# sdrobert/pydrobert-speech

Measured on AMD Instinct MI355X. Metric: frames/s (whole node) + HBM-roofline %, 40-mel fbank 16kHz 25/10ms, higher is better.
Workload: dtype f32

## Files before the change

include/pds_amd.h:

```cpp
#ifndef PDS_AMD_H
#define PDS_AMD_H

#include <stdint.h>

#ifdef __cplusplus
extern "C" {
#endif

#define PDS_OK 0
#define PDS_ERR_INVALID -1
#define PDS_ERR_HIP -2
#define PDS_ERR_NOMEM -3

int32_t pds_version(void);
int32_t pds_build_experiments(void);
const char *pds_last_error(void);
int32_t pds_device_count(void);

typedef struct pds_stft_desc {
  int32_t frame_length;
  int32_t frame_shift;
  int32_t dft_size;
  int32_t pad_left;
  int32_t num_filts;
  int32_t nnz;
  int32_t use_power;
  int32_t use_log;
  int32_t include_energy;
  int32_t reserved;
  double log_floor;
// ... 237 lines not shown
```

pydrobert-speech_amd/_native.py:

```python
import ctypes
import os
from ctypes import POINTER, Structure, c_char_p, c_double, c_int32, c_int64, c_void_p

_HERE = os.path.dirname(os.path.abspath(__file__))
LIB_PATH = os.environ.get("PDS_AMD_LIB") or os.path.join(_HERE, "csrc", "libpds_amd.so")

PDS_OK = 0


class NativeError(RuntimeError):
    """A call into libpds_amd.so failed"""


class StftDesc(Structure):
    _fields_ = [
        ("frame_length", c_int32),
        ("frame_shift", c_int32),
        ("dft_size", c_int32),
        ("pad_left", c_int32),
        ("num_filts", c_int32),
        ("nnz", c_int32),
        ("use_power", c_int32),
        ("use_log", c_int32),
        ("include_energy", c_int32),
# ... 41 lines not shown
    c_void_p, c_int64, c_int64, c_int64,
    c_void_p, c_void_p, c_int32,
    c_int32, c_int32,
    c_void_p, c_int64, c_int64, c_int64, c_int64,
    c_void_p,
]

_CMVN_ROWS_ARGS = [
    c_void_p, c_int64, c_void_p, c_void_p, c_int32, c_int32, c_int32,
    c_void_p, c_void_p, c_int64, c_void_p, c_void_p,
]

SIGNATURES = {
    "pds_version": (c_int32, []),
    "pds_build_experiments": (c_int32, []),
    "pds_last_error": (c_char_p, []),
    "pds_device_count": (c_int32, []),
    "pds_stft_plan_create": (
        c_int32,
        [POINTER(StftDesc), c_void_p, c_void_p, c_void_p, c_void_p, POINTER(c_void_p)],
    ),
    "pds_stft_plan_destroy": (None, [c_void_p]),
    "pds_stft_num_coeffs": (c_int32, [c_void_p]),
    "pds_stft_num_frames": (c_int64, [c_void_p, c_int64]),
    "pds_stft_plan_kernel_kind": (c_int32, [c_void_p]),
    "pds_stft_plan_filter_walk": (c_int32, [c_void_p]),
    "pds_stft_batch_f32": (c_int32, _BATCH_ARGS),
    "pds_stft_batch_f64": (c_int32, _BATCH_ARGS),
    "pds_stft_batch_f32_generic": (c_int32, _BATCH_ARGS),
    "pds_stft_plan_has_f64in": (c_int32, [c_void_p]),
# ... 148 lines not shown
```

pydrobert-speech_amd/csrc/stft_fast.hip:

```cpp
#include "stft_wave_launch.h"

namespace pds {

#if PDS_STAMPS
unsigned long long *g_stamp_buf = nullptr;
extern "C" __attribute__((visibility("default"))) void pds_debug_set_stamp_buffer(unsigned long long *d_buf) {
  g_stamp_buf = d_buf;
}
#endif

extern "C" __attribute__((visibility("default"))) int32_t pds_build_experiments(void) { return PDS_EXPERIMENTS ? 1 : 0; }

bool fast_has_f64in(const pds_stft_plan *plan) { return plan->fast.kind && fast_f64in_kind(plan->fast.kind); }

bool fast_has_fused_cmvn(const pds_stft_plan *plan) {
  const FastTables &ft = plan->fast;
  return ft.kind && ft.n2 == 16 && ((ft.n1 == 64 && ft.walk != 0) || (ft.n1 == 32 && (ft.walk == 1 || ft.walk == 3)));
}

bool fast_has_fused_deltas(const pds_stft_plan *plan) {
  const FastTables &ft = plan->fast;
  return ft.kind && fast_deltas_kind(ft.kind) && ft.rsn_rounds >= 1 && ft.rsn_rounds <= 2 &&
         (!plan->d.include_energy || ft.rs_eslot >= 0);
}

__global__ __launch_bounds__(1024) void chunk_prefix_kernel(const int64_t *nframes, int B, int groups, int64_t *prefix) {
// ... 382 lines not shown
```

pydrobert-speech_amd/csrc/stft_wave_kernel.h:

```cpp
#pragma once
#include <algorithm>
#include <atomic>
#include <cmath>
#include <cstdio>
#include <cstdlib>
#include <cstring>
#include <type_traits>
#include <vector>

#include "fft_inlane.h"
#include "mfma_front.h"
#include "rseg_tables.h"
#include "mseg_tables.h"
#include "pds_internal.h"

#include "stft_switches.h"

namespace pds {

__device__ __forceinline__ void keep_alive(float v) { asm volatile("" ::"v"(v)); }

struct FastParams {
  const void *sig;
  const int64_t *offsets, *lengths, *nframes, *row_off;
  void *out;
  int64_t out_stride;
  const float *win_lane;
  const float2 *tw_lane;
// ... 64 lines not shown
  typedef const T __attribute__((address_space(4))) *const_ptr;
  return *(const_ptr)(uintptr_t)ptr;
}

template <int CTRL>
__device__ __forceinline__ float dpp_add(float x) {
  return x + __int_as_float(__builtin_amdgcn_update_dpp(0, __float_as_int(x), CTRL, 0xf, 0xf, false));
}

__device__ __forceinline__ void wave_sync() {
  __builtin_amdgcn_fence(__ATOMIC_RELEASE, "wavefront");
  __builtin_amdgcn_wave_barrier();
  __builtin_amdgcn_fence(__ATOMIC_ACQUIRE, "wavefront");
}

#ifndef PDS_TWOPASS
#define PDS_TWOPASS 1
#endif
#ifndef PDS_LEAN_2048
#define PDS_LEAN_2048 1
#endif
constexpr bool lean_geometry(int n1, int n2) { return PDS_LEAN_2048 && n1 == 64 && n2 == 32; }
constexpr int wave_area_floats(int n1, int n2) {
  const int cols = (n1 - 1) / 2 + 1, groups = 64 / n2, one_pass = groups * cols * (n2 + 2) * 2;
  return (PDS_TWOPASS && n1 == 64 && n2 == 16) ? 2688 : lean_geometry(n1, n2) ? groups * cols * (n2 + 4) : one_pass;
}
constexpr int win_table_stride(int rows) { return ((rows + 3) & ~3) % 8 == 4 ? ((rows + 3) & ~3) : ((rows + 3) & ~3) + 4; }

template <int N1, int N2, int NROWS>
struct WaveGeom {
// ... 21 lines not shown
  static_assert(inl::is_pow2(N1) ? (FULL || N2 == 2 * COLS) : 600 % N1 == 0,
                "in-lane DFT sizes: 2^k, or a divisor of 600");
  static_assert(NROWS <= N1 && NROWS > 0, "rows");
};

constexpr int USLOTS = 4;

typedef float f32x4 __attribute__((ext_vector_type(4)));

template <int N1, int N2, int NROWS, int MAXWAVES, int MINW, bool ELL_LDS, bool PRE, int SEG = 0, int MF = 0,
          bool RSG = false, typename TIN = float, typename TOUT = float, int DLT = 0, bool STR = false, bool PF = false>
__global__ __launch_bounds__(MAXWAVES * 64, MINW) void stft_wave_kernel(const FastParams p) {
  static_assert(!PF || (DLT == 0 && !STR && MF == 0 && !PRE && std::is_same<TIN, float>::value && (N1 == 32 || N1 == 64) && N2 == 16),
                "prefetch: 16-lane power-of-two geometries, float32 samples, round-robin scheduling");
  constexpr bool STRETCH = DLT > 0 || STR;
  static_assert(!(STR && DLT > 0), "stretch scheduling is part of the fused-deltas launches already");
  static_assert(DLT == 0 || (DLT == 2 && N2 == 16 && RSG && std::is_same<TOUT, float>::value && MF == 0),
                "fused deltas: row-segment walk, float32 features");
  static_assert(MF == 0 || std::is_same<TIN, float>::value, "matrix-pipe front end: float32 samples");
  static_assert(std::is_same<TIN, float>::value || std::is_same<TIN, double>::value || std::is_same<TIN, int16_t>::value, "samples: float32, float64 or int16");
  using G = WaveGeom<N1, N2, NROWS>;
  constexpr int N = G::N, COLS = G::COLS, NREG = G::NREG, RS = G::RS, NB = G::NB, PSTR = G::PSTR;
  constexpr int MSLOTS = 2 * MF + 1;
  static_assert(MF == 0 || (N2 == 16 && N1 == 32 && MF == mfma_front_steps(NROWS)), "matrix-pipe front end: 32 x 16");
  static_assert(MF == 0 || 4 * MSLOTS * 64 <= G::EXCH_F2 * 2, "edge-frame gather reuses the exchange area");
  constexpr int NBP = (NB + 3) / 4 * 4;
  static_assert(!RSG || (G::GROUPS == 4 && ELL_LDS && !SEG && (NBP + 1) * 4 <= G::EXCH_F2 * 2),
                "row-segment walk: four frames per wave, tables in LDS");
  extern __shared__ __attribute__((aligned(16))) float smem[];
  const int lane = threadIdx.x & 63;
// ... 18 lines not shown
        t2 = fma(d, d, t2);
      }
    wstat[col] += t1;
    wstat[p.stat_cs + col] += t2;
  };
  float2 *exch = reinterpret_cast<float2 *>(wbase) + g * G::XROWS * RS;
  [[maybe_unused]] float *xf = wbase + g * (G::XROWS * G::RSF);
  float *Pg = wbase + g * PSTR;
  const int nthreads = p.waves * 64;
  float2 *sw_lds = reinterpret_cast<float2 *>(smem + p.waves * p.area_f);
  int *meta_lds = reinterpret_cast<int *>(sw_lds + N2);
  float *ellw_lds = reinterpret_cast<float *>(meta_lds + p.ell_meta_pad);
  constexpr bool TWCHAIN = (PF && PDS_PF_TW == 1) || (PAIR && (N1 == 32 || N1 == 64)) || (PDS_DLT_CHAIN && DLT > 0 && N1 == 32 && N2 == 16) || G::LEAN ||
                           (N1 == 64 && N2 == 16 && (SEG == 2 || PDS_LEAN_1024));
  constexpr bool WINLDS = PF && PDS_PF_WIN == 1;
  constexpr bool WINUSE = G::LEAN || (N1 == 64 && N2 == 16 && (SEG == 2 || PDS_LEAN_1024));
  constexpr int WSTR = win_table_stride(NROWS);
  [[maybe_unused]] float *win_lds = ellw_lds + (ELL_LDS ? p.ell_wfloats : 0);
  if constexpr (WINLDS || WINUSE) {
    const float *wsrc = TWCHAIN ? p.win_half : p.win_lane;
    for (int i = threadIdx.x; i < N2 * WSTR; i += p.waves * 64) {
      const int rr = i / WSTR, k = i - rr * WSTR;
      win_lds[i] = k < NROWS ? wsrc[rr * N1 + k] : 0.0f;
    }
  }
  if (threadIdx.x < N2) sw_lds[threadIdx.x] = p.tw_special[threadIdx.x];
  constexpr bool DYN = PDS_DYN && !STRETCH && !PF;
  [[maybe_unused]] int *ticket_lds = reinterpret_cast<int *>(smem + p.lds_ticket_off);
  if constexpr (DYN) {
    if (threadIdx.x == 0) *ticket_lds = p.waves;
  }
// ... 152 lines not shown
  };
  int nfr = 0, n = 0;
  int64_t sig_off = 0, out_row = 0;
  if (!STRETCH && b < p.num_utts) {
    nfr = (int)load_const(p.nframes + b);
    n = (int)load_const(p.lengths + b);
    sig_off = load_const(p.offsets + b);
    out_row = load_const(p.row_off + b);
  }
  constexpr int DR = 2;
  [[maybe_unused]] int left = 0, e_lo = 0, e_hi = 0, c_last = -1;
  [[maybe_unused]] bool piece_open = false, ran = false;
  [[maybe_unused]] float Wp[DR][4], Wc[DR][4], e_keep = 0.0f;
  if constexpr (STRETCH) {
    const int gw = wg * p.waves + wave, GW = (int)gridDim.x * p.waves;
    const int total = (int)load_const(p.chunk_prefix + p.num_utts);
    const int per = total / GW, rem = total - per * GW;
    const int pos = gw * per + (gw < rem ? gw : rem);
    left = per + (gw < rem ? 1 : 0);
    int lo = 0, hi = p.num_utts;
    while (left > 0 && hi - lo > 1) {
      const int mid = (lo + hi) >> 1;
      if ((int)load_const(p.chunk_prefix + mid) <= pos) lo = mid; else hi = mid;
    }
    b = lo;
    e_lo = left > 0 ? pos - (int)load_const(p.chunk_prefix + lo) : 0;
    chunk = 0;
#pragma unroll
    for (int rd = 0; rd < DR; ++rd)
#pragma unroll
      for (int q = 0; q < 4; ++q) Wp[rd][q] = Wc[rd][q] = 0.0f;
  }
  [[maybe_unused]] auto emit_rows = [&](const int ce, const float (&nx)[DR][4]) {
    if (p.dl_debug & 2) return;
    const int C = p.dl_inner;
    const int W = (p.dl_order + 1) * C, WS = (W + 3) & ~3;
    float *stage = wbase;
    wave_sync();
#pragma unroll
    for (int rd = 0; rd < DR; ++rd) {
      if (rd >= p.seg_rounds) break;
// ... 46 lines not shown
                const float4 val = *reinterpret_cast<const float4 *>(stage + q * WS + 4 * l);
                F4 o = {val.x, val.y, val.z, val.w};
                *reinterpret_cast<F4 *>(orow + (int64_t)q * p.out_stride + 4 * l) = o;
              }
          }
        }
      }
      if (tail) {
        const int q = tail == 1 ? lane : tail == 2 ? lane >> 1 : (lane * 11) >> 5;
        const int jj = lane - q * tail;
        if (q < fh && q < 4) orow[(int64_t)q * p.out_stride + 4 * full + jj] = stage[q * WS + 4 * full + jj];
      }
    }
    wave_sync();
  };
  [[maybe_unused]] unsigned long long st_acc[8] = {0, 0, 0, 0, 0, 0, 0, 0};
  [[maybe_unused]] unsigned long long st_prev = PDS_STAMPS ? __builtin_readcyclecounter() : 0;
  [[maybe_unused]] const unsigned long long st_loop = st_prev;
  while (STRETCH || b < p.num_utts) {
    if constexpr (STRETCH) {
      if (!piece_open) {
        if (left <= 0) break;
        nfr = (int)load_const(p.nframes + b);
        const int chunks_b = (nfr + G::GROUPS - 1) / G::GROUPS;
        if (e_lo >= chunks_b) {
          ++b;
          e_lo = 0;
          continue;
        }
        n = (int)load_const(p.lengths + b);
        sig_off = load_const(p.offsets + b);
        out_row = load_const(p.row_off + b);
        e_hi = e_lo + left < chunks_b ? e_lo + left : chunks_b;
        c_last = DLT > 0 ? (e_hi < chunks_b ? e_hi : chunks_b - 1) : e_hi - 1;
        chunk = DLT > 0 ? (e_lo > 0 ? e_lo - 1 : 0) : e_lo;
        piece_open = true;
        ran = false;
      }
      if constexpr (STR) {
        if (ran) ++chunk;
        ran = true;
      }
      if (chunk > c_last) {
        if (DLT > 0 && c_last < e_hi) {
          float nx[DR][4];
#pragma unroll
          for (int rd = 0; rd < DR; ++rd)
#pragma unroll
            for (int q = 0; q < 4; ++q) nx[rd][q] = Wc[rd][3];
          emit_rows(c_last, nx);
        }
        if constexpr (STATS) {
          if (stats_on) {
            wave_sync();
            double *dst = p.stat_part + ((int64_t)(wg * p.waves + wave) + b) * (2 * p.stat_c);
            for (int c = lane; c < p.stat_c; c += 64) {
              dst[c] = wstat[c];
              dst[p.stat_c + c] = wstat[p.stat_cs + c];
              wstat[c] = 0.0;
              wstat[p.stat_cs + c] = 0.0;
            }
            wave_sync();
          }
        }
        left -= e_hi - e_lo;
        ++b;
        e_lo = 0;
        piece_open = false;
        continue;
      }
    }
    int nchunk = chunk + p.step_chunks, nb = b + p.step_utts;
    if (nchunk >= p.chunks_per_utt) {
      nchunk -= p.chunks_per_utt;
      ++nb;
    }
    const int pb = nb < p.num_utts ? nb : b;
    const int tb = chunk * G::GROUPS;
    if constexpr (DYN) {
      if (p.dyn) fetch_ticket();
// ... 29 lines not shown
      const float *base = pf_ready ? static_cast<const float *>(p.sig) + (sig_off_nx + s02) : p.win_lane;
      const float *xp2 = base + (pf_ready ? pf_lane : r);
#pragma unroll
      for (int n1 = 0; n1 < NROWS; ++n1) {
        pfv[n1] = xp2[n1 * N2];
#if PDS_PF_ILV > 0
        __builtin_amdgcn_sched_group_barrier(0x020, 1, 0);
        __builtin_amdgcn_sched_group_barrier(0x002, PDS_PF_ILV, 0);
#endif
      }
    };
    const TIN *x = static_cast<const TIN *>(p.sig) + sig_off;
    const int start0 = tb * S - p.pad_left;
    bool valid = true;
    float energy = 0.0f;
    const float2 sw = sw_lds[r];
    [[maybe_unused]] float even_sum, odd_sum, Ar[COLS], Ai[COLS];
    if constexpr (MF > 0) {
      int fstart[4];
#pragma unroll
      for (int fg = 0; fg < 4; ++fg) fstart[fg] = start0 + fg * S;
      int wmode = 0;
      if (!(tb + 4 <= nfr && start0 >= (PRE ? 1 : 0) && start0 + 3 * S + NROWS * 16 <= n)) {
        valid = tb + g < nfr;
#pragma unroll
        for (int fg = 0; fg < 4; ++fg) {
          const int st = (tb + fg < nfr ? tb + fg : nfr - 1) * S - p.pad_left;
          fstart[fg] = st;
          int mode = (st < (PRE ? 1 : 0) || st + NROWS * 16 > n) ? 1 : 0;
          if (st < -n || st + L > 2 * n) mode = 2;
          wmode = mode > wmode ? mode : wmode;
// ... 116 lines not shown
        for (int v = 0; v < 4; ++v) {
          float2 val;
          val.x = accR[fg][v] * mtwr[v] - accI[fg][v] * mtwi[v];
          val.y = accR[fg][v] * mtwi[v] + accI[fg][v] * mtwr[v];
          if (v < 3 || g != 3) {
            mine[fg * COLS * RS + v * RS] = val;
          } else {
            row0[fg * COLS * RS * 2] = accR[fg][3];
            row0[fg * COLS * RS * 2 + 16] = accI[fg][3];
          }
        }
      }
    } else {
      int start = start0 + __mul24(g, S);
      int wmode = 0;
      if (!(PF && pf_ready) && !(tb + G::GROUPS <= nfr && start0 >= (PRE ? 1 : 0) &&
            start0 + (G::GROUPS - 1) * S + LOADSPAN <= n)) {
        valid = tb + g < nfr;
        start = (valid ? tb + g : nfr - 1) * S - p.pad_left;
        int mode = 0;
        if (start < (PRE ? 1 : 0) || start + LOADSPAN > n) mode = 1;
        if (start < -n || start + L > 2 * n) mode = 2;
        wmode = __builtin_amdgcn_readfirstlane(__any(mode == 2) ? 2 : (__any(mode == 1) ? 1 : 0));
      }

      float a[N1];
      if (PF && pf_ready) {
#pragma unroll
        for (int n1 = 0; n1 < NROWS; ++n1) a[n1] = pfv[n1];
      } else if (wmode == 0) {
        const TIN *xp = x + (start + r);
        if constexpr (PAIR) {
          typedef double D2 __attribute__((ext_vector_type(2), aligned(8)));
          const TIN *xq = x + (start + 2 * r);
          constexpr int NP = (NROWS + 1) / 2;
          D2 w2[NP];
          [[maybe_unused]] double before = 0.0;
#pragma unroll
          for (int j = 0; j < NP; ++j) w2[j] = *reinterpret_cast<const D2 *>(xq + 32 * j);
          if constexpr (PRE) {
            if (r == 0) before = xq[-1];
          }
// ... 123 lines not shown
                i = (int)reflect_index((int64_t)i, (int64_t)n);
              }
              if constexpr (!F64S) {
                v = (float)x[i];
                if (PRE && i > 0) v = preemph_sample(v, (float)x[i - 1], p.preemph);
              } else {
                TIN w = x[i];
                if (PRE && i > 0) w = preemph_sample(w, x[i - 1], (TIN)p.preemph_d);
                v = (float)w;
              }
            }
            tmp[(n1 - base) * 64 + lane] = v;
          }
          wave_sync();
#pragma unroll
          for (int n1 = base; n1 < top; ++n1) a[n1] = tmp[(n1 - base) * 64 + lane];
          wave_sync();
        });
      }
      if (p.include_energy) {
        int lim = L - rho;
        asm volatile("" : "+v"(lim));
#pragma unroll
        for (int n1 = 0; n1 < NROWS; ++n1) {
          const float v = (n1 < N1 / 2 || n1 * N2 < lim) ? a[n1] : 0.0f;
          energy = fmaf(v, v, energy);
        }
      }
      PDS_STAMP(0, 0);
      PDS_STAMP(1, 1);
      PDS_PHASE(4);
      if constexpr (WINLDS) {
#pragma unroll
        for (int n1 = 0; n1 < NROWS; ++n1) a[n1] = window_mul<N1>(n1, a[n1], wl[n1]);
      } else if constexpr (WINUSE) {
        const float4 *w4 = reinterpret_cast<const float4 *>(win_lds + rho * WSTR);
#pragma unroll
        for (int j = 0; j < (NROWS + 3) / 4; ++j) {
          const float4 w = w4[j];
          const float wv[4] = {w.x, w.y, w.z, w.w};
#pragma unroll
          for (int u = 0; u < 4; ++u)
            if (4 * j + u < NROWS) a[4 * j + u] = window_mul<N1>(4 * j + u, a[4 * j + u], wv[u]);
        }
      } else {
#pragma unroll
        for (int n1 = 0; n1 < NROWS; ++n1) a[n1] = window_mul<N1>(n1, a[n1], win[n1]);
      }
      if constexpr (PF) fetch_next_record();
#pragma unroll
      for (int n1 = NROWS; n1 < N1; ++n1) a[n1] = 0.0f;

      if constexpr (PDS_ABLATE & 2) {
        even_sum = a[0];
        odd_sum = a[1];
#pragma unroll
        for (int k = 0; k < COLS; ++k) {
          Ar[k] = a[2 * k];
// ... 264 lines not shown
        if constexpr (G::FULL && PDS_MIRROR_REBASE) {
          float *const Pa = Pw + kk * PB, *const Pm = Pw + (N1 - kk) * PB;
#pragma unroll
          for (int k2 = 0; k2 < N2 / 2; ++k2) Pa[N1 * k2 * PB] = pw[q][k2];
#pragma unroll
          for (int k2 = N2 / 2; k2 < N2; ++k2) Pm[N1 * (N2 - 1 - k2) * PB] = pw[q][k2];
        } else
#pragma unroll
        for (int k2 = 0; k2 < N2; ++k2) {
          const int bin = (k2 < N2 / 2) ? kk + N1 * k2 : N - kk - N1 * k2;
          Pw[(live ? bin : PDUMP) * PB] = pw[q][k2];
        }
      }
    }
    if constexpr (G::DIST) {
      const bool has = r <= N2 / 2 && (N1 % 2 == 0 || r % 2 == 0);
      Pw[(has ? r * N1 / 2 : PDUMP) * PB] = sp0;
      Pw[(has ? (N2 - r) * N1 / 2 : PDUMP) * PB] = sp1;
    }
    if constexpr (RSG) {
      constexpr int PADF = (NBP - NB) * 4;
      wbase[NB * 4 + (lane < PADF ? lane : PADF - 1)] = 0.0f;
    } else {
#pragma unroll
      for (int j0 = 0; j0 < PSTR - NB; j0 += N2) {
        const int j = j0 + r;
        Pg[NB + (j < PSTR - NB ? j : PSTR - NB - 1)] = 0.0f;
      }
    }
    TOUT *obase = static_cast<TOUT *>(p.out) + (out_row + tb) * p.out_stride;
    const unsigned lane_off = (unsigned)(g * (int)p.out_stride + col0);
    if (p.include_energy) {
      if constexpr (MF == 0) {
        energy = dpp_add<0xB1>(energy);
        energy = dpp_add<0x4E>(energy);
        energy = dpp_add<0x141>(energy);
        if constexpr (N2 >= 16) energy = dpp_add<0x140>(energy);
        if constexpr (N2 >= 32) energy += __shfl_xor(energy, 16, 64);
        if constexpr (N2 == 64) energy += __shfl_xor(energy, 32, 64);
      }
      float e = energy * p.inv_L;
      if (!use_power) e = __builtin_amdgcn_sqrtf(e);
      if (p.use_log) e = floor_log(e, p.log_floor);
      if (DLT == 0 && valid && r == 0) {
        unsigned off = (lane_off - col0) * (unsigned)sizeof(TOUT);
        asm("" : "+v"(off));
        *reinterpret_cast<TOUT *>(reinterpret_cast<char *>(obase) + off) = (TOUT)e;
      }
      if constexpr (DLT > 0) e_keep = e;
      if constexpr (STATS) {
        if (stats_on) {
          const float e4[4] = {__int_as_float(__builtin_amdgcn_readlane(__float_as_int(e), 0)),
                               __int_as_float(__builtin_amdgcn_readlane(__float_as_int(e), 16)),
                               __int_as_float(__builtin_amdgcn_readlane(__float_as_int(e), 32)),
                               __int_as_float(__builtin_amdgcn_readlane(__float_as_int(e), 48))};
          if (lane == 0) stat_add4(0, e4, nfr - tb);
        }
      }
    }
    PDS_STAMP(4, 0);
// ... 71 lines not shown
      if (steps & 1u) step();
      float acc = (acc0 + acc1) + (acc2 + acc3);
      if (p.use_log) acc = floor_log(acc, p.log_floor);
      if constexpr (PDS_ABLATE & 64) {
        keep_alive(acc);
      } else {
        const unsigned byte_off = (lane_off + (unsigned)(meta >> 16) - 1u) * (unsigned)sizeof(TOUT);
        if (valid && meta >= 0x10000)
          *reinterpret_cast<TOUT *>(reinterpret_cast<char *>(obase) + byte_off) = (TOUT)acc;
      }
    };
    if constexpr (RSG) {
      const float4 *P4 = reinterpret_cast<const float4 *>(wbase);
      const int t4n = p.seg_len >> 2;
      char *const orow0 = reinterpret_cast<char *>(obase);
      const int64_t row_bytes = p.out_stride * (int64_t)sizeof(TOUT);
      auto round_body = [&](const int rd, float (&logged)[4]) {
        const int4 rec = reinterpret_cast<const int4 *>(meta_lds)[rd * 64 + lane];
        const float4 *prow = reinterpret_cast<const float4 *>(reinterpret_cast<const char *>(P4) + rec.x);
        const float4 *wrow = reinterpret_cast<const float4 *>(ellw_lds) + __mul24(rd, t4n) * 64 + lane;
        float a0 = 0.0f, a1 = 0.0f, a2 = 0.0f, a3 = 0.0f;
        auto quad = [&](int t4) {
          const float4 w = wrow[t4 * 64];
          const float4 x0 = prow[4 * t4], x1 = prow[4 * t4 + 1], x2 = prow[4 * t4 + 2], x3 = prow[4 * t4 + 3];
          a0 = fmaf(w.x, x0.x, a0);
          a1 = fmaf(w.x, x0.y, a1);
          a2 = fmaf(w.x, x0.z, a2);
          a3 = fmaf(w.x, x0.w, a3);
          a0 = fmaf(w.y, x1.x, a0);
          a1 = fmaf(w.y, x1.y, a1);
          a2 = fmaf(w.y, x1.z, a2);
// ... 41 lines not shown
                     : "+v"(a0), "+v"(a1), "+v"(a2), "+v"(a3) : "v"(m1), "v"(m2));
#else
        a0 = fmaf(shl(a0, inl::Int<0x101>{}), m1, a0);
        a1 = fmaf(shl(a1, inl::Int<0x101>{}), m1, a1);
        a2 = fmaf(shl(a2, inl::Int<0x101>{}), m1, a2);
        a3 = fmaf(shl(a3, inl::Int<0x101>{}), m1, a3);
        a0 = fmaf(shl(a0, inl::Int<0x102>{}), m2, a0);
        a1 = fmaf(shl(a1, inl::Int<0x102>{}), m2, a1);
        a2 = fmaf(shl(a2, inl::Int<0x102>{}), m2, a2);
        a3 = fmaf(shl(a3, inl::Int<0x102>{}), m2, a3);
#endif
        const int coff = rec.w;
        const float vals[4] = {a0, a1, a2, a3};
        unsigned off = (unsigned)coff;
        auto put = [&](const int gg, const float v) {
          if (DLT == 0 && coff >= 0 && gg < frames_here) {
            asm("" : "+v"(off));
            *reinterpret_cast<TOUT *>(orow0 + gg * row_bytes + off) = (TOUT)v;
          }
          logged[gg] = v;
        };
        if (p.use_log) {
#pragma unroll
          for (int gg = 0; gg < 4; ++gg) put(gg, floor_log(vals[gg], p.log_floor));
        } else {
#pragma unroll
          for (int gg = 0; gg < 4; ++gg) put(gg, vals[gg]);
        }
        if constexpr (STATS) {
          if (stats_on && coff >= 0) stat_add4(coff / (int)sizeof(TOUT), logged, frames_here);
        }
// ... 227 lines not shown
```

pydrobert-speech_amd/csrc/stft_wave_launch.h:

```cpp
#pragma once
#include "stft_wave_kernel.h"

namespace pds {


constexpr bool fast_f64in_kind(int n) { return n == 256 || n == 512 || n == 1024 || n == 2048; }

constexpr bool fast_deltas_kind(int n) { return n == 512 || n == 1024; }


template <int N1, int N2, int NROWS, int MINW>
int32_t launch_wave(const pds_stft_plan *plan, const BatchArgs &a) {
  using G = WaveGeom<N1, N2, NROWS>;
#ifndef PDS_DLT_MINW
#define PDS_DLT_MINW 3
#endif
  constexpr int DMINW = (N1 == 64 && N2 == 16) ? 2 : MINW > PDS_DLT_MINW ? PDS_DLT_MINW : MINW;
  constexpr int CU_WAVES_STFT = 4 * MINW;
  constexpr int F64_MINW = (N1 == 64 && N2 == 16) ? 2 : MINW, F64_WAVES = 4 * F64_MINW;
  const int CU_WAVES = a.dl_K > 0 ? 4 * DMINW : a.in_f64 ? F64_WAVES : CU_WAVES_STFT;
  const FastTables &ft = plan->fast;
  FastParams p;
  p.sig = a.d_signal;
  p.offsets = a.d_offsets;
// ... 56 lines not shown
  int walk = 0;
  const bool dl = a.dl_K > 0 && ft.rsn_rounds > 0;
  constexpr bool PFG = (N1 == 32 || N1 == 64) && N2 == 16;
  const char *pf_env = std::getenv("PDS_STFT_PF");
  constexpr bool PF_PRODUCT = N1 == 64 && N2 == 16;
  [[maybe_unused]] constexpr bool PF_MSEG = false;
  constexpr bool MSEG3 = N1 == 64 && N2 == 16;
  constexpr int MS_WAVES = MSEG3 ? 12 : 4 * MINW, MS_MINW = MSEG3 ? 3 : MINW;
  static_assert(!MSEG3 || !PDS_LEAN_1024 || MINW == 3, "the 64 x 16 geometry is instantiated for three waves per SIMD (stft_geoms.def)");
  const bool pf_ok = (PDS_EXPERIMENTS || PF_PRODUCT) && PFG && !pre && !a.in_f64 && !a.in_i16 && !a.stretch && a.dl_K == 0 &&
                     ft.d_win_half && ft.d_tw_seed && !(pf_env && pf_env[0] == '0');
  constexpr int PF_WSTR = ((NROWS + 3) & ~3) % 8 == 4 ? ((NROWS + 3) & ~3) : ((NROWS + 3) & ~3) + 4;
  const size_t pf_extra = (PDS_PF_WIN == 1) ? (size_t)N2 * PF_WSTR * 4 : 0;
  const size_t lean_extra = LEAN_ALL ? (size_t)N2 * win_table_stride(NROWS) * 4 : 0;
  const size_t mseg3_extra = LEAN_ALL ? 0 : (size_t)N2 * win_table_stride(NROWS) * 4;
  constexpr bool MSG = G::GROUPS == 4 && inl::is_pow2(N1);
  constexpr bool SEGOK = G::GROUPS == 4 || (inl::is_pow2(N1) && N2 >= 32);
  for (int cand = (G::GROUPS == 4) ? (dl ? 2 : ft.walk) : (SEGOK && ft.walk == 1 ? 1 : 0); cand >= 0 && !in_lds; --cand) {
    if (cand == 3 && (!MSG || ft.ms_rounds == 0 || pre || a.in_f64 || a.in_i16)) continue;
    if ((cand == 2 && !dl && ft.rs_rounds == 0) || (cand == 1 && (ft.seg_rounds == 0 || pre || a.in_f64 || a.in_i16))) continue;
    const int meta_ints = cand == 3 ? ft.ms_meta_ints : cand == 2 ? (dl ? ft.rsn_rounds : ft.rs_rounds) * 64 : cand == 1 ? ft.seg_meta_ints : ft.ell_slots * N2;
    const int meta_pad = cand == 2 ? meta_ints * 4 : (std::max(meta_ints, USLOTS * N2) + 3) / 4 * 4;
    const size_t fixed = (size_t)N2 * 8 + (size_t)meta_pad * 4 + (cand == 2 && pf_ok ? pf_extra : 0) + lean_extra +
                         (cand == 3 && MSEG3 ? mseg3_extra : 0);
    const size_t table_bytes = (size_t)(cand == 3 ? ft.ms_wfloats : cand == 2 ? (dl ? ft.rsn_wfloats : ft.rs_wfloats) : cand == 1 ? ft.seg_wfloats : ft.ell_wfloats) * 4;
    if (cand == 1 && (size_t)G::GROUPS * G::PSTR * 4 + (size_t)ft.seg_rounds * 64 * 4 * G::GROUPS > per_wave) continue;
    if (cand == 3 && (size_t)G::GROUPS * G::PSTR * 4 + (size_t)ft.ms_slots * 64 > per_wave) continue;
    const size_t area_c = (cand == 3 && MSEG3)
                              ? std::max((size_t)G::XMIN_F * 4, (size_t)G::GROUPS * G::PSTR * 4 + (size_t)ft.ms_slots * 64)
                              : per_wave;
    const int ms_shapes[5][2] = {{12, 1}, {11, 1}, {10, 1}, {9, 1}, {8, 1}};
    const int (*try_shapes)[2] = (cand == 3 && MSEG3) ? ms_shapes : shapes;
    for (int si = 0; si < ((cand == 3 && MSEG3) ? 5 : 4); ++si) {
      const int *shape = try_shapes[si];
      if (shape[0] * (area_c + stat_pw) + fixed + table_bytes + 48 <= lds_cu / shape[1]) {
        waves = shape[0];
        wgs_per_cu = shape[1];
        in_lds = true;
        area_bytes = area_c;
// ... 15 lines not shown
      p.seg_rounds = ft.seg_rounds;
      p.seg_len = ft.seg_len;
    } else if (in_lds && cand == 2) {
      p.ell_w = dl ? ft.d_rsn_w : ft.d_rs_w;
      p.ell_meta = dl ? ft.d_rsn_meta : ft.d_rs_meta;
      p.ell_wfloats = dl ? ft.rsn_wfloats : ft.rs_wfloats;
      p.seg_rounds = dl ? ft.rsn_rounds : ft.rs_rounds;
      p.seg_len = dl ? ft.rsn_len : ft.rs_len;
    }
    if (in_lds) walk = cand;
  }
#ifdef PDS_FORCE_WAVES
  if (in_lds && PDS_FORCE_WAVES <= CU_WAVES / 2) waves = PDS_FORCE_WAVES, wgs_per_cu = 2;
#endif
  const size_t fixed = (size_t)N2 * 8 + (size_t)p.ell_meta_pad * 4 + (walk == 2 && in_lds && pf_ok ? pf_extra : 0) + lean_extra +
                       (walk == 3 && in_lds && MSEG3 ? mseg3_extra : 0);
  const size_t table_bytes = (size_t)p.ell_wfloats * 4;
  if (a.in_i16 && !in_lds) {
    set_error("stft_batch_i16in: not served for this plan (filter table outside LDS)");
    return PDS_ERR_INVALID;
  }
  if (pre && !in_lds) return launch_stft_generic_f32(plan, a);
  p.preemph = (float)a.preemph;
  p.preemph_d = a.preemph;
  p.waves = waves;
  p.mf_tab = ft.d_mf_tab;
#if PDS_STAMPS
  p.stamps = g_stamp_buf;
#else
  p.stamps = nullptr;
#endif
// ... 40 lines not shown
  }
#if PDS_EXPERIMENTS
  if constexpr (PFG) {
    if (pf_ok && in_lds && !mf && (rsg || seg || (mseg && !PF_MSEG))) {
      pf_used = true;
      kern = rsg    ? stft_wave_kernel<N1, N2, NROWS, CU_WAVES_K, MINW, true, false, 0, 0, W4, float, float, 0, false, PFG>
             : mseg ? stft_wave_kernel<N1, N2, NROWS, CU_WAVES_K, MINW, true, false, MSG ? 2 : 0, 0, false, float, float, 0, false, PFG>
                    : stft_wave_kernel<N1, N2, NROWS, CU_WAVES_K, MINW, true, false, SEGOK ? 1 : 0, 0, false, float, float, 0, false, PFG>;
      p.win_half = ft.d_win_half;
      p.tw_seed = (const float2 *)ft.d_tw_seed;
    }
  }
#endif
  bool str_used = false;
  if constexpr (inl::is_pow2(N1))
  if (a.stretch && !pre && !a.in_f64 && !a.in_i16 && a.dl_K == 0 && !mf && a.d_chunk_prefix && in_lds) {
    str_used = true;
    kern = rsg      ? stft_wave_kernel<N1, N2, NROWS, CU_WAVES_K, MINW, true, false, 0, 0, W4, float, float, 0, true>
           : mseg   ? stft_wave_kernel<N1, N2, NROWS, MS_WAVES, MS_MINW, true, false, MSG ? 2 : 0, 0, false, float, float, 0, true>
           : seg    ? stft_wave_kernel<N1, N2, NROWS, CU_WAVES_K, MINW, true, false, SEGOK ? 1 : 0, 0, false, float, float, 0, true>
                    : stft_wave_kernel<N1, N2, NROWS, CU_WAVES_K, MINW, true, false, 0, 0, false, float, float, 0, true>;
    p.chunk_prefix = a.d_chunk_prefix;
  }
  int strx_which = -1;
  if constexpr (W4 && (N1 == 32 || N1 == 64) && N2 == 16) {
    if (a.stretch && (pre || a.in_i16) && !a.in_f64 && a.dl_K == 0 && !mf && a.d_chunk_prefix && in_lds && rsg && !a.d_stat_part) {
      using I = int16_t;
      str_used = true;
      kern = a.in_i16 ? (pre ? stft_wave_kernel<N1, N2, NROWS, CU_WAVES_K, MINW, true, true, 0, 0, true, I, float, 0, true>
                             : stft_wave_kernel<N1, N2, NROWS, CU_WAVES_K, MINW, true, false, 0, 0, true, I, float, 0, true>)
                      : stft_wave_kernel<N1, N2, NROWS, CU_WAVES_K, MINW, true, true, 0, 0, true, float, float, 0, true>;
      p.chunk_prefix = a.d_chunk_prefix;
      strx_which = a.in_i16 ? (pre ? 38 : 37) : 36;
    }
  }
  if (a.d_stat_part) {
    if (!str_used || !in_lds || walk == 0 || G::GROUPS != 4 || (rsg && MINW > 2)) {
      set_error("stft_cmvn_batch: not served for this plan and call (needs a 16-lane power-of-two geometry, a segment "
                "walk with its tables and the waves' sums in LDS, float32 samples, no fused pre-emphasis)");
      return PDS_ERR_INVALID;
    }
// ... 32 lines not shown
      if (a.in_f64 || a.out_f64 || a.d_stat_part) {
        set_error("stft_batch_i16in: float32 features, no fused CMVN sums");
        return PDS_ERR_INVALID;
      }
      mf = false;
      kern = pre ? (rsg ? stft_wave_kernel<N1, N2, NROWS, CU_WAVES_K, MINW, true, true, false, 0, W4, int16_t, float>
                        : stft_wave_kernel<N1, N2, NROWS, CU_WAVES_K, MINW, true, true, false, 0, false, int16_t, float>)
                 : (rsg ? stft_wave_kernel<N1, N2, NROWS, CU_WAVES_K, MINW, true, false, false, 0, W4, int16_t, float>
                        : stft_wave_kernel<N1, N2, NROWS, CU_WAVES_K, MINW, true, false, false, 0, false, int16_t, float>);
      i16_which = 32 + (pre ? 2 : 0) + (rsg ? 1 : 0);
    } else {
      set_error("stft_batch_i16in: no fused int16-input kernel for this transform size");
      return PDS_ERR_INVALID;
    }
  }
  int dl_which = -1;
  if (a.dl_K > 0) {
    constexpr bool DELTAS = fast_deltas_kind(N1 * N2) && G::GROUPS == 4;
    if constexpr (DELTAS) {
      const int staged = ((a.dl_K + 1) * (plan->d.num_filts + (plan->d.include_energy ? 1 : 0)) + 3) / 4 * 16 + 64;
      if (!in_lds || !rsg || !dl || ft.rsn_rounds > 2 || (plan->d.include_energy && ft.rs_eslot < 0) || a.out_f64 ||
          staged > G::EXCH_F2 * 2) {
        set_error("stft_deltas_batch: not served for this plan and call (needs the row-segment filter walk with at "
                  "most two rounds in LDS and float32 features)");
        return PDS_ERR_INVALID;
      }
      mf = false;
      using D = double;
      using I = int16_t;
      kern = a.in_f64 ? (pre ? stft_wave_kernel<N1, N2, NROWS, 4 * DMINW, DMINW, true, true, false, 0, true, D, float, 2>
// ... 12 lines not shown
      for (int j = 0; j < 9; ++j) p.dl_f2[j] = a.dl_K > 1 ? (float)a.dl_taps[5 + j] : 0.0f;
      p.dl_inner = plan->d.num_filts + (plan->d.include_energy ? 1 : 0);
      p.dl_eslot = plan->d.include_energy ? ft.rs_eslot : -1;
      p.chunk_prefix = a.d_chunk_prefix;
#if defined(PDS_DL_DEBUG_SWITCH) && PDS_DL_DEBUG_SWITCH
      p.dl_debug = std::getenv("PDS_DL_DEBUG") ? std::atoi(std::getenv("PDS_DL_DEBUG")) : 0;
#else
      p.dl_debug = 0;
#endif
    } else {
      set_error("stft_deltas_batch: no fused kernel for this transform size");
      return PDS_ERR_INVALID;
    }
  }
  constexpr int kDevices = 64;
  static std::atomic<size_t> attr_smem[kDevices][40];
  const int which = strx_which >= 0  ? strx_which
                    : dl_which >= 0    ? dl_which
                    : f64_which >= 0 ? f64_which
                    : i16_which >= 0 ? i16_which
                    : pf_used        ? (rsg ? 27 : mseg ? 30 : 31)
                    : str_used       ? 22 + (rsg ? 0 : mseg ? 1 : seg ? 2 : 3)
                    : mseg           ? 20
                                     : (pre ? (rsg ? 5 : 2) : rsg ? 4 : seg ? 3 : (in_lds ? 1 : 0)) + (mf ? 6 : 0);
  const bool cached = plan->device >= 0 && plan->device < kDevices;
  if (!cached || smem > attr_smem[plan->device][which].load(std::memory_order_relaxed)) {
    PDS_HIP(hipFuncSetAttribute((const void *)kern, hipFuncAttributeMaxDynamicSharedMemorySize,
                                (int)smem));
    if (cached) attr_smem[plan->device][which].store(smem, std::memory_order_relaxed);
  }
  int64_t grid = (int64_t)ft.num_cus * wgs_per_cu;
  const int64_t need = (chunks * a.B + waves - 1) / waves;
  if (grid > need) grid = need;
  const int64_t grid_waves = grid * waves;
  p.step_utts = (int)(grid_waves / chunks);
  p.step_chunks = (int)(grid_waves % chunks);
  if (a.dl_K > 0 || str_used) {
    grid = std::min<int64_t>((int64_t)ft.num_cus * wgs_per_cu, std::max<int64_t>(1, (chunks * a.B + 4 * waves - 1) / (4 * waves)));
    if (!a.prefix_prepared) {
      const int32_t rc_prefix = launch_chunk_prefix(a.d_nframes, a.B, G::GROUPS, a.d_chunk_prefix, a.stream);
      if (rc_prefix != PDS_OK) return rc_prefix;
    }
  }
  if (a.grid_waves_out) *a.grid_waves_out = (int32_t)(grid * waves);
  hipLaunchKernelGGL(kern, dim3((unsigned)grid), dim3(waves * 64), smem, a.stream, p);
  PDS_HIP(hipGetLastError());
  return PDS_OK;
}

}
```

Before: 4.079 billion.

## Add frame-run STFT path reusing overlapping sample rows across consecutive frames

Adds a specialised path for the 512-point (32x16) geometry with 25 rows. Each of the four lane groups now processes a contiguous run of frames instead of interleaved frames. When consecutive frames are regular and the shift equals a whole number of rows, the overlapping 15 rows of raw samples are shifted in registers and only the new rows are loaded from global memory. It also adds a grid-mode chunk assignment that skips the chunk-prefix kernel and its binary search when stretch scheduling is off. The cost is extra register pressure from the raw buffer, a different output stride pattern, and a new kernel variant selected by default, plus a debug query for which kernel ran.

```diff
diff --git a/include/pds_amd.h b/include/pds_amd.h
--- a/include/pds_amd.h
+++ b/include/pds_amd.h
@@ -14,6 +14,7 @@
 
 int32_t pds_version(void);
 int32_t pds_build_experiments(void);
+int32_t pds_debug_last_stft_kernel(void);
 const char *pds_last_error(void);
 int32_t pds_device_count(void);
 
diff --git a/pydrobert-speech_amd/_native.py b/pydrobert-speech_amd/_native.py
--- a/pydrobert-speech_amd/_native.py
+++ b/pydrobert-speech_amd/_native.py
@@ -79,6 +79,7 @@
 SIGNATURES = {
     "pds_version": (c_int32, []),
     "pds_build_experiments": (c_int32, []),
+    "pds_debug_last_stft_kernel": (c_int32, []),
     "pds_last_error": (c_char_p, []),
     "pds_device_count": (c_int32, []),
     "pds_stft_plan_create": (
diff --git a/pydrobert-speech_amd/csrc/frame_runs.h b/pydrobert-speech_amd/csrc/frame_runs.h
--- /dev/null
+++ b/pydrobert-speech_amd/csrc/frame_runs.h
@@ -0,0 +1,43 @@
+#pragma once
+
+#if defined(__HIPCC__)
+#define PDS_RUNS_FN __host__ __device__ inline
+#else
+#define PDS_RUNS_FN inline
+#endif
+
+namespace pds {
+namespace runs {
+
+struct Piece {
+  int f0;
+  int F;
+  int K;
+};
+
+PDS_RUNS_FN Piece piece_of(int e_lo, int e_hi, int nfr) {
+  Piece p;
+  p.f0 = 4 * e_lo;
+  const int f1 = 4 * e_hi < nfr ? 4 * e_hi : nfr;
+  p.F = f1 - p.f0;
+  p.K = (p.F + 3) >> 2;
+  return p;
+}
+
+PDS_RUNS_FN int frame_of(const Piece &p, int g, int j) { return g * p.K + j; }
+PDS_RUNS_FN bool exists(const Piece &p, int g, int j) { return g * p.K + j < p.F; }
+PDS_RUNS_FN int stand_in(const Piece &p) { return p.f0 + p.F - 1; }
+
+PDS_RUNS_FN int start_of(int frame, int S, int pad_left) { return frame * S - pad_left; }
+
+PDS_RUNS_FN bool regular(const Piece &p, int j, int S, int pad_left, int span, int n) {
+  return 3 * p.K + j < p.F && start_of(p.f0 + j, S, pad_left) >= 0 &&
+         start_of(p.f0 + 3 * p.K + j, S, pad_left) + span <= n;
+}
+
+PDS_RUNS_FN bool full_load(int j, bool regular_now, bool regular_before) {
+  return j == 0 || !regular_now || !regular_before;
+}
+
+}
+}
diff --git a/pydrobert-speech_amd/csrc/stft_fast.hip b/pydrobert-speech_amd/csrc/stft_fast.hip
--- a/pydrobert-speech_amd/csrc/stft_fast.hip
+++ b/pydrobert-speech_amd/csrc/stft_fast.hip
@@ -10,6 +10,11 @@
 #endif
 
 extern "C" __attribute__((visibility("default"))) int32_t pds_build_experiments(void) { return PDS_EXPERIMENTS ? 1 : 0; }
+
+std::atomic<int> g_last_stft_kernel{-1};
+extern "C" __attribute__((visibility("default"))) int32_t pds_debug_last_stft_kernel(void) {
+  return g_last_stft_kernel.load(std::memory_order_relaxed);
+}
 
 bool fast_has_f64in(const pds_stft_plan *plan) { return plan->fast.kind && fast_f64in_kind(plan->fast.kind); }
 
diff --git a/pydrobert-speech_amd/csrc/stft_wave_kernel.h b/pydrobert-speech_amd/csrc/stft_wave_kernel.h
--- a/pydrobert-speech_amd/csrc/stft_wave_kernel.h
+++ b/pydrobert-speech_amd/csrc/stft_wave_kernel.h
@@ -12,6 +12,7 @@
 #include "mfma_front.h"
 #include "rseg_tables.h"
 #include "mseg_tables.h"
+#include "frame_runs.h"
 #include "pds_internal.h"
 
 #include "stft_switches.h"
@@ -106,6 +107,12 @@
   __builtin_amdgcn_fence(__ATOMIC_ACQUIRE, "wavefront");
 }
 
+template <typename TIN, typename TOUT>
+constexpr bool frame_runs_kind(int n1, int n2, int rows, int minw, bool pre, int seg, int mf, bool rsg, int dlt, bool str) {
+  return n1 == 32 && n2 == 16 && rows == 25 && minw == 4 && !pre && seg == 0 && mf == 0 && rsg && dlt == 0 && str &&
+         !std::is_same<TIN, double>::value && std::is_same<TOUT, float>::value;
+}
+
 #ifndef PDS_TWOPASS
 #define PDS_TWOPASS 1
 #endif
@@ -157,6 +164,8 @@
   static_assert(!PF || (DLT == 0 && !STR && MF == 0 && !PRE && std::is_same<TIN, float>::value && (N1 == 32 || N1 == 64) && N2 == 16),
                 "prefetch: 16-lane power-of-two geometries, float32 samples, round-robin scheduling");
   constexpr bool STRETCH = DLT > 0 || STR;
+  constexpr bool RUN = frame_runs_kind<TIN, TOUT>(N1, N2, NROWS, MINW, PRE, SEG, MF, RSG, DLT, STR);
+  constexpr int RUN_D = RUN ? NROWS - 15 : 0;
   static_assert(!(STR && DLT > 0), "stretch scheduling is part of the fused-deltas launches already");
   static_assert(DLT == 0 || (DLT == 2 && N2 == 16 && RSG && std::is_same<TOUT, float>::value && MF == 0),
                 "fused deltas: row-segment walk, float32 features");
@@ -205,7 +214,7 @@
   constexpr bool TWCHAIN = (PF && PDS_PF_TW == 1) || (PAIR && (N1 == 32 || N1 == 64)) || (PDS_DLT_CHAIN && DLT > 0 && N1 == 32 && N2 == 16) || G::LEAN ||
                            (N1 == 64 && N2 == 16 && (SEG == 2 || PDS_LEAN_1024));
   constexpr bool WINLDS = PF && PDS_PF_WIN == 1;
-  constexpr bool WINUSE = G::LEAN || (N1 == 64 && N2 == 16 && (SEG == 2 || PDS_LEAN_1024));
+  constexpr bool WINUSE = RUN || G::LEAN || (N1 == 64 && N2 == 16 && (SEG == 2 || PDS_LEAN_1024));
   constexpr int WSTR = win_table_stride(NROWS);
   [[maybe_unused]] float *win_lds = ellw_lds + (ELL_LDS ? p.ell_wfloats : 0);
   if constexpr (WINLDS || WINUSE) {
@@ -388,17 +397,24 @@
   [[maybe_unused]] float Wp[DR][4], Wc[DR][4], e_keep = 0.0f;
   if constexpr (STRETCH) {
     const int gw = wg * p.waves + wave, GW = (int)gridDim.x * p.waves;
-    const int total = (int)load_const(p.chunk_prefix + p.num_utts);
+    const bool grid_mode = RUN && p.chunk_prefix == nullptr;
+    const int total = grid_mode ? p.num_utts * p.chunks_per_utt : (int)load_const(p.chunk_prefix + p.num_utts);
     const int per = total / GW, rem = total - per * GW;
     const int pos = gw * per + (gw < rem ? gw : rem);
     left = per + (gw < rem ? 1 : 0);
     int lo = 0, hi = p.num_utts;
-    while (left > 0 && hi - lo > 1) {
+    while (!grid_mode && left > 0 && hi - lo > 1) {
       const int mid = (lo + hi) >> 1;
       if ((int)load_const(p.chunk_prefix + mid) <= pos) lo = mid; else hi = mid;
     }
     b = lo;
-    e_lo = left > 0 ? pos - (int)load_const(p.chunk_prefix + lo) : 0;
+    e_lo = left > 0 && !grid_mode ? pos - (int)load_const(p.chunk_prefix + lo) : 0;
+    if constexpr (RUN) {
+      if (grid_mode) {
+        b = (int)((unsigned)pos / (unsigned)p.chunks_per_utt);
+        e_lo = pos - b * p.chunks_per_utt;
+      }
+    }
     chunk = 0;
 #pragma unroll
     for (int rd = 0; rd < DR; ++rd)
@@ -475,6 +491,10 @@
     }
     wave_sync();
   };
+  [[maybe_unused]] runs::Piece pc_run = {0, 0, 0};
+  [[maybe_unused]] int run_start = 0;
+  [[maybe_unused]] bool run_reg_before = false;
+  [[maybe_unused]] float raw[RUN ? NROWS : 1];
   [[maybe_unused]] unsigned long long st_acc[8] = {0, 0, 0, 0, 0, 0, 0, 0};
   [[maybe_unused]] unsigned long long st_prev = PDS_STAMPS ? __builtin_readcyclecounter() : 0;
   [[maybe_unused]] const unsigned long long st_loop = st_prev;
@@ -484,7 +504,18 @@
         if (left <= 0) break;
         nfr = (int)load_const(p.nframes + b);
         const int chunks_b = (nfr + G::GROUPS - 1) / G::GROUPS;
-        if (e_lo >= chunks_b) {
+        if constexpr (RUN) {
+          const int span_b = p.chunk_prefix == nullptr ? p.chunks_per_utt : chunks_b;
+          const int take = left < span_b - e_lo ? left : span_b - e_lo;
+          left -= take;
+          if (e_lo >= chunks_b) {
+            ++b;
+            e_lo = 0;
+            continue;
+          }
+          e_hi = e_lo + take < chunks_b ? e_lo + take : chunks_b;
+        }
+        if (!RUN && e_lo >= chunks_b) {
           ++b;
           e_lo = 0;
           continue;
@@ -492,9 +523,17 @@
         n = (int)load_const(p.lengths + b);
         sig_off = load_const(p.offsets + b);
         out_row = load_const(p.row_off + b);
-        e_hi = e_lo + left < chunks_b ? e_lo + left : chunks_b;
+        if constexpr (!RUN) e_hi = e_lo + left < chunks_b ? e_lo + left : chunks_b;
         c_last = DLT > 0 ? (e_hi < chunks_b ? e_hi : chunks_b - 1) : e_hi - 1;
         chunk = DLT > 0 ? (e_lo > 0 ? e_lo - 1 : 0) : e_lo;
+        if constexpr (RUN) {
+          pc_run = runs::piece_of(e_lo, e_hi, nfr);
+          chunk = 0;
+          c_last = pc_run.K - 1;
+          run_reg_before = false;
+          const int gk = __mul24(g, pc_run.K);
+          run_start = __mul24(pc_run.f0 + gk, S) - p.pad_left;
+        }
         piece_open = true;
         ran = false;
       }
@@ -524,7 +563,7 @@
             wave_sync();
           }
         }
-        left -= e_hi - e_lo;
+        if constexpr (!RUN) left -= e_hi - e_lo;
         ++b;
         e_lo = 0;
         piece_open = false;
@@ -584,7 +623,9 @@
     const int start0 = tb * S - p.pad_left;
     bool valid = true;
     float energy = 0.0f;
-    const float2 sw = sw_lds[r];
+    int r_sw = r;
+    if constexpr (RUN) asm volatile("" : "+v"(r_sw));
+    const float2 sw = sw_lds[r_sw];
     [[maybe_unused]] float even_sum, odd_sum, Ar[COLS], Ai[COLS];
     if constexpr (MF > 0) {
       int fstart[4];
@@ -731,7 +772,23 @@
     } else {
       int start = start0 + __mul24(g, S);
       int wmode = 0;
-      if (!(PF && pf_ready) && !(tb + G::GROUPS <= nfr && start0 >= (PRE ? 1 : 0) &&
+      [[maybe_unused]] bool run_reg = false, run_full = true;
+      if constexpr (RUN) {
+        run_reg = runs::regular(pc_run, chunk, S, p.pad_left, LOADSPAN, n);
+        run_full = runs::full_load(chunk, run_reg, run_reg_before) || S != RUN_D * N2;
+        run_reg_before = run_reg;
+        start = run_start;
+        run_start += S;
+        if (!run_reg) {
+          valid = runs::exists(pc_run, g, chunk);
+          start = runs::start_of(valid ? pc_run.f0 + runs::frame_of(pc_run, g, chunk) : runs::stand_in(pc_run), S, p.pad_left);
+          int mode = 0;
+          if (start < 0 || start + LOADSPAN > n) mode = 1;
+          if (start < -n || start + L > 2 * n) mode = 2;
+          wmode = __builtin_amdgcn_readfirstlane(__any(mode == 2) ? 2 : (__any(mode == 1) ? 1 : 0));
+        }
+      }
+      if (!RUN && !(PF && pf_ready) && !(tb + G::GROUPS <= nfr && start0 >= (PRE ? 1 : 0) &&
             start0 + (G::GROUPS - 1) * S + LOADSPAN <= n)) {
         valid = tb + g < nfr;
         start = (valid ? tb + g : nfr - 1) * S - p.pad_left;
@@ -742,7 +799,18 @@
       }
 
       float a[N1];
-      if (PF && pf_ready) {
+      if (RUN && wmode == 0) {
+        const TIN *xp = x + (start + r);
+        if (run_full) {
+#pragma unroll
+          for (int n1 = 0; n1 < NROWS - RUN_D; ++n1) raw[RUN ? n1 : 0] = (float)xp[n1 * N2];
+        } else {
+#pragma unroll
+          for (int n1 = 0; n1 < NROWS - RUN_D; ++n1) raw[RUN ? n1 : 0] = raw[RUN ? n1 + RUN_D : 0];
+        }
+#pragma unroll
+        for (int n1 = NROWS - RUN_D; n1 < NROWS; ++n1) raw[RUN ? n1 : 0] = (float)xp[n1 * N2];
+      } else if (PF && pf_ready) {
 #pragma unroll
         for (int n1 = 0; n1 < NROWS; ++n1) a[n1] = pfv[n1];
       } else if (wmode == 0) {
@@ -896,7 +964,7 @@
           }
           wave_sync();
 #pragma unroll
-          for (int n1 = base; n1 < top; ++n1) a[n1] = tmp[(n1 - base) * 64 + lane];
+          for (int n1 = base; n1 < top; ++n1) (RUN ? raw[RUN ? n1 : 0] : a[n1]) = tmp[(n1 - base) * 64 + lane];
           wave_sync();
         });
       }
@@ -905,7 +973,7 @@
         asm volatile("" : "+v"(lim));
 #pragma unroll
         for (int n1 = 0; n1 < NROWS; ++n1) {
-          const float v = (n1 < N1 / 2 || n1 * N2 < lim) ? a[n1] : 0.0f;
+          const float v = (n1 < N1 / 2 || n1 * N2 < lim) ? (RUN ? raw[RUN ? n1 : 0] : a[n1]) : 0.0f;
           energy = fmaf(v, v, energy);
         }
       }
@@ -923,7 +991,7 @@
           const float wv[4] = {w.x, w.y, w.z, w.w};
 #pragma unroll
           for (int u = 0; u < 4; ++u)
-            if (4 * j + u < NROWS) a[4 * j + u] = window_mul<N1>(4 * j + u, a[4 * j + u], wv[u]);
+            if (4 * j + u < NROWS) a[4 * j + u] = window_mul<N1>(4 * j + u, RUN ? raw[RUN ? 4 * j + u : 0] : a[4 * j + u], wv[u]);
         }
       } else {
 #pragma unroll
@@ -1218,9 +1286,11 @@
       }
     }
     if constexpr (G::DIST) {
-      const bool has = r <= N2 / 2 && (N1 % 2 == 0 || r % 2 == 0);
-      Pw[(has ? r * N1 / 2 : PDUMP) * PB] = sp0;
-      Pw[(has ? (N2 - r) * N1 / 2 : PDUMP) * PB] = sp1;
+      int r_sp = r;
+      if constexpr (RUN) asm volatile("" : "+v"(r_sp));
+      const bool has = r_sp <= N2 / 2 && (N1 % 2 == 0 || r_sp % 2 == 0);
+      Pw[(has ? r_sp * N1 / 2 : PDUMP) * PB] = sp0;
+      Pw[(has ? (N2 - r_sp) * N1 / 2 : PDUMP) * PB] = sp1;
     }
     if constexpr (RSG) {
       constexpr int PADF = (NBP - NB) * 4;
@@ -1232,7 +1302,7 @@
         Pg[NB + (j < PSTR - NB ? j : PSTR - NB - 1)] = 0.0f;
       }
     }
-    TOUT *obase = static_cast<TOUT *>(p.out) + (out_row + tb) * p.out_stride;
+    TOUT *obase = static_cast<TOUT *>(p.out) + (out_row + (RUN ? pc_run.f0 + chunk : tb)) * p.out_stride;
     const unsigned lane_off = (unsigned)(g * (int)p.out_stride + col0);
     if (p.include_energy) {
       if constexpr (MF == 0) {
@@ -1247,7 +1317,10 @@
       if (!use_power) e = __builtin_amdgcn_sqrtf(e);
       if (p.use_log) e = floor_log(e, p.log_floor);
       if (DLT == 0 && valid && r == 0) {
-        unsigned off = (lane_off - col0) * (unsigned)sizeof(TOUT);
+        int g_e = g;
+        if constexpr (RUN) asm volatile("" : "+v"(g_e));
+        unsigned off = RUN ? (unsigned)__mul24(g_e, pc_run.K) * (unsigned)p.out_stride * (unsigned)sizeof(TOUT)
+                           : (lane_off - col0) * (unsigned)sizeof(TOUT);
         asm("" : "+v"(off));
         *reinterpret_cast<TOUT *>(reinterpret_cast<char *>(obase) + off) = (TOUT)e;
       }
@@ -1349,7 +1422,7 @@
       const float4 *P4 = reinterpret_cast<const float4 *>(wbase);
       const int t4n = p.seg_len >> 2;
       char *const orow0 = reinterpret_cast<char *>(obase);
-      const int64_t row_bytes = p.out_stride * (int64_t)sizeof(TOUT);
+      const int64_t row_bytes = p.out_stride * (int64_t)sizeof(TOUT) * (RUN ? pc_run.K : 1);
       auto round_body = [&](const int rd, float (&logged)[4]) {
         const int4 rec = reinterpret_cast<const int4 *>(meta_lds)[rd * 64 + lane];
         const float4 *prow = reinterpret_cast<const float4 *>(reinterpret_cast<const char *>(P4) + rec.x);
@@ -1421,7 +1494,7 @@
         const float vals[4] = {a0, a1, a2, a3};
         unsigned off = (unsigned)coff;
         auto put = [&](const int gg, const float v) {
-          if (DLT == 0 && coff >= 0 && gg < frames_here) {
+          if (DLT == 0 && coff >= 0 && (RUN ? runs::exists(pc_run, gg, chunk) : gg < frames_here)) {
             asm("" : "+v"(off));
             *reinterpret_cast<TOUT *>(orow0 + gg * row_bytes + off) = (TOUT)v;
           }
diff --git a/pydrobert-speech_amd/csrc/stft_wave_launch.h b/pydrobert-speech_amd/csrc/stft_wave_launch.h
--- a/pydrobert-speech_amd/csrc/stft_wave_launch.h
+++ b/pydrobert-speech_amd/csrc/stft_wave_launch.h
@@ -3,6 +3,8 @@
 
 namespace pds {
 
+
+extern std::atomic<int> g_last_stft_kernel;
 
 constexpr bool fast_f64in_kind(int n) { return n == 256 || n == 512 || n == 1024 || n == 2048; }
 
@@ -94,6 +96,12 @@
   const size_t pf_extra = (PDS_PF_WIN == 1) ? (size_t)N2 * PF_WSTR * 4 : 0;
   const size_t lean_extra = LEAN_ALL ? (size_t)N2 * win_table_stride(NROWS) * 4 : 0;
   const size_t mseg3_extra = LEAN_ALL ? 0 : (size_t)N2 * win_table_stride(NROWS) * 4;
+  constexpr bool RUNG = frame_runs_kind<float, float>(N1, N2, NROWS, MINW, false, 0, 0, true, 0, true);
+  const char *run_env = std::getenv("PDS_STFT_RUNS");
+  const bool run_ok = RUNG && !pre && !a.in_f64 && !a.out_f64 && a.dl_K == 0 && !a.d_stat_part &&
+                      (!a.stretch || a.d_chunk_prefix) && a.max_frames * a.out_stride < 0x3fffffff &&
+                      !(run_env && run_env[0] == '0');
+  const size_t run_extra = run_ok ? (size_t)N2 * win_table_stride(NROWS) * 4 : 0;
   constexpr bool MSG = G::GROUPS == 4 && inl::is_pow2(N1);
   constexpr bool SEGOK = G::GROUPS == 4 || (inl::is_pow2(N1) && N2 >= 32);
   for (int cand = (G::GROUPS == 4) ? (dl ? 2 : ft.walk) : (SEGOK && ft.walk == 1 ? 1 : 0); cand >= 0 && !in_lds; --cand) {
@@ -102,7 +110,7 @@
     const int meta_ints = cand == 3 ? ft.ms_meta_ints : cand == 2 ? (dl ? ft.rsn_rounds : ft.rs_rounds) * 64 : cand == 1 ? ft.seg_meta_ints : ft.ell_slots * N2;
     const int meta_pad = cand == 2 ? meta_ints * 4 : (std::max(meta_ints, USLOTS * N2) + 3) / 4 * 4;
     const size_t fixed = (size_t)N2 * 8 + (size_t)meta_pad * 4 + (cand == 2 && pf_ok ? pf_extra : 0) + lean_extra +
-                         (cand == 3 && MSEG3 ? mseg3_extra : 0);
+                         (cand == 3 && MSEG3 ? mseg3_extra : 0) + (cand == 2 ? run_extra : 0);
     const size_t table_bytes = (size_t)(cand == 3 ? ft.ms_wfloats : cand == 2 ? (dl ? ft.rsn_wfloats : ft.rs_wfloats) : cand == 1 ? ft.seg_wfloats : ft.ell_wfloats) * 4;
     if (cand == 1 && (size_t)G::GROUPS * G::PSTR * 4 + (size_t)ft.seg_rounds * 64 * 4 * G::GROUPS > per_wave) continue;
     if (cand == 3 && (size_t)G::GROUPS * G::PSTR * 4 + (size_t)ft.ms_slots * 64 > per_wave) continue;
@@ -148,7 +156,7 @@
   if (in_lds && PDS_FORCE_WAVES <= CU_WAVES / 2) waves = PDS_FORCE_WAVES, wgs_per_cu = 2;
 #endif
   const size_t fixed = (size_t)N2 * 8 + (size_t)p.ell_meta_pad * 4 + (walk == 2 && in_lds && pf_ok ? pf_extra : 0) + lean_extra +
-                       (walk == 3 && in_lds && MSEG3 ? mseg3_extra : 0);
+                       (walk == 3 && in_lds && MSEG3 ? mseg3_extra : 0) + (walk == 2 && in_lds ? run_extra : 0);
   const size_t table_bytes = (size_t)p.ell_wfloats * 4;
   if (a.in_i16 && !in_lds) {
     set_error("stft_batch_i16in: not served for this plan (filter table outside LDS)");
@@ -219,7 +227,7 @@
 #endif
   bool str_used = false;
   if constexpr (inl::is_pow2(N1))
-  if (a.stretch && !pre && !a.in_f64 && !a.in_i16 && a.dl_K == 0 && !mf && a.d_chunk_prefix && in_lds) {
+  if (a.stretch && !pre && !a.in_f64 && !a.in_i16 && a.dl_K == 0 && !mf && a.d_chunk_prefix && in_lds && !(RUNG && rsg)) {
     str_used = true;
     kern = rsg      ? stft_wave_kernel<N1, N2, NROWS, CU_WAVES_K, MINW, true, false, 0, 0, W4, float, float, 0, true>
            : mseg   ? stft_wave_kernel<N1, N2, NROWS, MS_WAVES, MS_MINW, true, false, MSG ? 2 : 0, 0, false, float, float, 0, true>
@@ -229,7 +237,8 @@
   }
   int strx_which = -1;
   if constexpr (W4 && (N1 == 32 || N1 == 64) && N2 == 16) {
-    if (a.stretch && (pre || a.in_i16) && !a.in_f64 && a.dl_K == 0 && !mf && a.d_chunk_prefix && in_lds && rsg && !a.d_stat_part) {
+    if (a.stretch && (pre || a.in_i16) && !a.in_f64 && a.dl_K == 0 && !mf && a.d_chunk_prefix && in_lds && rsg && !a.d_stat_part &&
+        !(RUNG && !pre)) {
       using I = int16_t;
       str_used = true;
       kern = a.in_i16 ? (pre ? stft_wave_kernel<N1, N2, NROWS, CU_WAVES_K, MINW, true, true, 0, 0, true, I, float, 0, true>
@@ -292,6 +301,17 @@
       return PDS_ERR_INVALID;
     }
   }
+  int run_which = -1;
+  if constexpr (RUNG) {
+    if (run_ok && in_lds && rsg && !mf) {
+      str_used = true;
+      strx_which = f64_which = i16_which = -1;
+      kern = a.in_i16 ? stft_wave_kernel<N1, N2, NROWS, CU_WAVES_K, MINW, true, false, 0, 0, true, int16_t, float, 0, true>
+                      : stft_wave_kernel<N1, N2, NROWS, CU_WAVES_K, MINW, true, false, 0, 0, true, float, float, 0, true>;
+      p.chunk_prefix = a.stretch ? a.d_chunk_prefix : nullptr;
+      run_which = a.in_i16 ? 40 : 39;
+    }
+  }
   int dl_which = -1;
   if (a.dl_K > 0) {
     constexpr bool DELTAS = fast_deltas_kind(N1 * N2) && G::GROUPS == 4;
@@ -334,8 +354,9 @@
     }
   }
   constexpr int kDevices = 64;
-  static std::atomic<size_t> attr_smem[kDevices][40];
-  const int which = strx_which >= 0  ? strx_which
+  static std::atomic<size_t> attr_smem[kDevices][42];
+  const int which = run_which >= 0   ? run_which
+                    : strx_which >= 0  ? strx_which
                     : dl_which >= 0    ? dl_which
                     : f64_which >= 0 ? f64_which
                     : i16_which >= 0 ? i16_which
@@ -357,12 +378,13 @@
   p.step_chunks = (int)(grid_waves % chunks);
   if (a.dl_K > 0 || str_used) {
     grid = std::min<int64_t>((int64_t)ft.num_cus * wgs_per_cu, std::max<int64_t>(1, (chunks * a.B + 4 * waves - 1) / (4 * waves)));
-    if (!a.prefix_prepared) {
+    if (!a.prefix_prepared && !(run_which >= 0 && !a.stretch)) {
       const int32_t rc_prefix = launch_chunk_prefix(a.d_nframes, a.B, G::GROUPS, a.d_chunk_prefix, a.stream);
       if (rc_prefix != PDS_OK) return rc_prefix;
     }
   }
   if (a.grid_waves_out) *a.grid_waves_out = (int32_t)(grid * waves);
+  g_last_stft_kernel.store(which, std::memory_order_relaxed);
   hipLaunchKernelGGL(kern, dim3((unsigned)grid), dim3(waves * 64), smem, a.stream, p);
   PDS_HIP(hipGetLastError());
   return PDS_OK;
```

Result: slower. 3.763 billion (-7.7%).
